# xingchensong/TouchNet

Hardware: AMD Instinct MI355X
Metric: audio+text tokens/sec/node (packed seq, full train step) + step MFU (higher is better)
Workload: dtype bf16

## Files before the change

### touchnet_amd/csrc/common.h

```cpp
#pragma once
#include <hip/hip_runtime.h>
#include <stdint.h>

#define TN_OK 0
#define TN_EINVAL (-22)

#define TN_LAUNCH_CHECK()                                   \
  do {                                                      \
    hipError_t e__ = hipGetLastError();                     \
    if (e__ != hipSuccess) return (int)e__;                 \
  } while (0)

namespace tn {

typedef uint16_t bf16_t;

typedef __attribute__((ext_vector_type(8))) __bf16 bf16x8_t;
typedef __attribute__((ext_vector_type(16))) float f32x16_t;
typedef __attribute__((ext_vector_type(4))) float f32x4_t;

__device__ __forceinline__ float bf2f(bf16_t v) { return __uint_as_float(((uint32_t)v) << 16); }

typedef __attribute__((ext_vector_type(2))) __bf16 bf16x2_t;

// ... 69 lines not shown
      f[2 * i + 1] = __uint_as_float(w[i] & 0xffff0000u);
    }
  }
  __device__ __forceinline__ void pack(const float (&f)[8]) {
    raw.x = pack2bf(f[0], f[1]);
    raw.y = pack2bf(f[2], f[3]);
    raw.z = pack2bf(f[4], f[5]);
    raw.w = pack2bf(f[6], f[7]);
  }
};
template <> struct Vec16<float> {
  static constexpr int N = 4;
  float4 raw;
  __device__ __forceinline__ void load(const float* p) { raw = *reinterpret_cast<const float4*>(p); }
  __device__ __forceinline__ void store(float* p) const { *reinterpret_cast<float4*>(p) = raw; }
  __device__ __forceinline__ void unpack(float (&f)[4]) const {
    f[0] = raw.x; f[1] = raw.y; f[2] = raw.z; f[3] = raw.w;
  }
  __device__ __forceinline__ void pack(const float (&f)[4]) { raw = make_float4(f[0], f[1], f[2], f[3]); }
};

__device__ __forceinline__ float wave_sum(float v) {
#pragma unroll
  for (int o = 32; o > 0; o >>= 1) v += __shfl_xor(v, o, 64);
  return v;
}
__device__ __forceinline__ float wave_max(float v) {
#pragma unroll
  for (int o = 32; o > 0; o >>= 1) v = fmaxf(v, __shfl_xor(v, o, 64));
  return v;
}

__device__ __forceinline__ float block_sum(float v, float* sm) {
  v = wave_sum(v);
  const int lane = threadIdx.x & 63, w = threadIdx.x >> 6, nw = (blockDim.x + 63) >> 6;
  __syncthreads();
  if (lane == 0) sm[w] = v;
  __syncthreads();
  float r = 0.f;
  for (int i = 0; i < nw; ++i) r += sm[i];
  return r;
}
__device__ __forceinline__ float block_max(float v, float* sm) {
  v = wave_max(v);
  const int lane = threadIdx.x & 63, w = threadIdx.x >> 6, nw = (blockDim.x + 63) >> 6;
  __syncthreads();
  if (lane == 0) sm[w] = v;
  __syncthreads();
  float r = sm[0];
  for (int i = 1; i < nw; ++i) r = fmaxf(r, sm[i]);
  return r;
}

}
```

### touchnet_amd/csrc/gemm.hip

```cpp
#include <stdlib.h>

#include <type_traits>
#include <utility>

#include "common.h"

namespace tn {
namespace gemm {

constexpr int BM = 256, BN = 256;
constexpr int SLOT = 32768;
constexpr int LDS_BYTES = 5 * SLOT;
constexpr int NT = 512;
constexpr int MAXSEG = 3;

typedef __attribute__((address_space(3))) void* lds_ptr_t;
typedef __attribute__((ext_vector_type(2))) uint32_t u32x2_t;
typedef __attribute__((ext_vector_type(4))) uint32_t u32x4_t;

struct Seg {
  const bf16_t* A;
  const bf16_t* B;
  long long lda, ldb;
  int K;
  int pad_;
};

struct Grp {
  bf16_t* C;
  long long ldc;
  int M, N, nbm, nbn;
  int start;
  int stages;
};

constexpr int EPI_PLAIN = 0, EPI_GROUPED = 1, EPI_SWIGLU_FWD = 2, EPI_SWIGLU_BWD = 3, EPI_BIASG = 4, EPI_ROPE = 5;
constexpr int EPI_GELU_FWD = 6, EPI_GELU_BWD = 7;

struct Params {
  Seg seg[MAXSEG];
  int nseg;
  int M, N;
  bf16_t* C;
  bf16_t* Ct;
  const bf16_t* bias;
  long long ldc, ldct;
  int accumulate;
  const bf16_t* addend;
  long long ldadd;
  int nbm, nbn;
  int stages;
  int splitk, kchunk;
  float* ws;
  int tile0, ntiles;
  int c_f32;
  Grp grp[MAXSEG];
  int ngrp;
  bf16_t* C2;
  bf16_t* C3;
  const bf16_t* E1;
  const bf16_t* E2;
  long long lde;
  bf16_t* bias_out;
  float* bias_ws;
  const bf16_t* rope_cos;
  const bf16_t* rope_sin;
  int rope_d;
};

__device__ __forceinline__ void tile_of_block(int bid, int nbm, int nbn, int& tm, int& tn) {
  const int total = nbm * nbn;
  const int xcd = bid & 7, local = bid >> 3;
  const int q = total >> 3, r = total & 7;
  const int vid = (xcd < r ? xcd * (q + 1) : r * (q + 1) + (xcd - r) * q) + local;
  constexpr int GM = 8;
  const int per_group = GM * nbn;
  const int g = vid / per_group, w = vid - g * per_group;
  const int gm = min(GM, nbm - g * GM);
  tm = g * GM + w % gm;
  tn = w / gm;
}

typedef f32x16_t Acc[4][2];

constexpr int kPieceB[4] = {0, 2, 4, 6}, kPieceA[4] = {14, 18, 22, 26};
static_assert(kPieceB[3] < kPieceA[0], "every B piece is issued before the first A piece");

template <bool IS_A> constexpr int piece_at(int pos) {
  for (int i = 0; i < 4; ++i)
    if ((IS_A ? kPieceA[i] : kPieceB[i]) == pos) return i;
  return -1;
}
constexpr int early_piece_count() {
  int n = 0;
  for (int i = 0; i < 4; ++i) n += (kPieceB[i] < 8) + (kPieceA[i] < 8);
  return n;
}

template <bool KMAJ, bool M16 = false>
struct Stream {
  __amdgpu_buffer_rsrc_t rs;
  int soff;
  int step;
  int left;
  int seg;
  int ld2;
  int voff[4];

  __device__ __forceinline__ void set_voff(int wave, int lane) {
    if constexpr (!KMAJ) {
#pragma unroll
      for (int q = 0; q < 4; ++q) {
        const int row = wave * 32 + q * 8 + (lane >> 3);
        voff[q] = row * ld2 + (((lane & 7) ^ ((row >> 1) & 7)) << 4);
      }
    } else {
#pragma unroll
      for (int q = 0; q < 4; ++q) {
        const int k = wave * 8 + q * 2 + (lane >> 5);
        const int u = lane & 31;
// ... 192 lines not shown
        if (sB.seg + 1 < p.nseg) open_b(sB.seg + 1);
        else if (++kb < mine) open_b(0);
        else sB.kill(p.C);
      }
    };
    auto piece_a = [&](int slot, int q) {
      __builtin_amdgcn_raw_ptr_buffer_load_lds(sA.rs, (lds_ptr_t)(smem + slot * SLOT + wave * 4096 + q * 1024), 16,
                                               sA.voff[q], sA.soff, 0, 0);
    };
    auto piece_b = [&](int slot, int q) {
      __builtin_amdgcn_raw_ptr_buffer_load_lds(sB.rs, (lds_ptr_t)(smem + slot * SLOT + wave * 4096 + q * 1024), 16,
                                               sB.voff[q], sB.soff, 0, 0);
    };
    open_a(0);
    open_b(0);

    Reader<AK, 4> ra(lane, wr * 128);
    Reader<BK, 2> rb(lane, wc * 64);

    Acc acc;
    auto zero_acc = [&]() {
#pragma unroll
      for (int i = 0; i < 4; ++i)
#pragma unroll
        for (int j = 0; j < 2; ++j)
#pragma unroll
          for (int r = 0; r < 16; ++r) acc[i][j][r] = 0.f;
    };
    zero_acc();

    Frags<AK, 4> ae, ao;
    Frags<BK, 2> be, bo;

#define TN_PIN() __builtin_amdgcn_sched_barrier(0)
    auto read_frag = [&](auto QC, auto FC, int sa, int sb, Frags<AK, 4>& a, Frags<BK, 2>& b) {
      constexpr int Q = decltype(QC)::value, F = decltype(FC)::value;
      if constexpr (F < 2) rb.template read<Q, F>(smem, sb * SLOT, b);
      else ra.template read<Q, F - 2>(smem, sa * SLOT, a);
    };
    auto read_all = [&](auto QC, int sa, int sb, Frags<AK, 4>& a, Frags<BK, 2>& b) {
      read_frag(QC, std::integral_constant<int, 0>{}, sa, sb, a, b);
      read_frag(QC, std::integral_constant<int, 1>{}, sa, sb, a, b);
      read_frag(QC, std::integral_constant<int, 2>{}, sa, sb, a, b);
      read_frag(QC, std::integral_constant<int, 3>{}, sa, sb, a, b);
      read_frag(QC, std::integral_constant<int, 4>{}, sa, sb, a, b);
      read_frag(QC, std::integral_constant<int, 5>{}, sa, sb, a, b);
    };
    auto mma = [&](const Frags<AK, 4>& a, const Frags<BK, 2>& b, int i, int j) {
      acc[i][j] = __builtin_amdgcn_mfma_f32_32x32x16_bf16(b.v[j], a.v[i], acc[i][j], 0, 0, 0);
    };

    float bsum = 0.f;
    bool bias_on = false;
    auto bias_accum = [&](const Frags<AK, 4>& a) {
      auto add = [&](const bf16x8_t& v) {
        const u32x4_t w = __builtin_bit_cast(u32x4_t, v);
        bsum += ((__uint_as_float(w.x << 16) + __uint_as_float(w.x & 0xffff0000u)) +
                 (__uint_as_float(w.y << 16) + __uint_as_float(w.y & 0xffff0000u))) +
                ((__uint_as_float(w.z << 16) + __uint_as_float(w.z & 0xffff0000u)) +
                 (__uint_as_float(w.w << 16) + __uint_as_float(w.w & 0xffff0000u)));
      };
      if (wc == 0) add(a.v[0]);
      else if (wc == 1) add(a.v[1]);
      else if (wc == 2) add(a.v[2]);
      else add(a.v[3]);
    };

    auto quarter = [&](auto NQC, auto P0C, const Frags<AK, 4>& ca, const Frags<BK, 2>& cb, Frags<AK, 4>& na,
                       Frags<BK, 2>& nb, int nsa, int nsb, int dst_b, int dst_a) {
      constexpr int P0 = decltype(P0C)::value;
      if constexpr (EPI == EPI_BIASG) {
        if (bias_on) bias_accum(ca);
        TN_PIN();
      }
      auto step = [&](auto MC) {
        constexpr int m = decltype(MC)::value;
        mma(ca, cb, m >> 1, m & 1);
        TN_PIN();
        if constexpr (m < 6) {
          read_frag(NQC, std::integral_constant<int, m>{}, nsa, nsb, na, nb);
          TN_PIN();
        }
        constexpr int pb = P0 < 0 ? -1 : piece_at<false>(P0 + m);
        constexpr int pa = P0 < 0 ? -1 : piece_at<true>(P0 + m);
        if constexpr (pb >= 0) {
          piece_b(dst_b, pb);
          if constexpr (pb == 3) adv_b();
          TN_PIN();
        }
        if constexpr (pa >= 0) {
          piece_a(dst_a, pa);
          if constexpr (pa == 3) adv_a();
          TN_PIN();
        }
      };
      step(std::integral_constant<int, 0>{});
      step(std::integral_constant<int, 1>{});
      step(std::integral_constant<int, 2>{});
      step(std::integral_constant<int, 3>{});
      step(std::integral_constant<int, 4>{});
      step(std::integral_constant<int, 5>{});
      step(std::integral_constant<int, 6>{});
      step(std::integral_constant<int, 7>{});
    };
    auto early_pieces = [&](int dst_b, int dst_a) {
      auto one = [&](auto MC) {
        constexpr int m = decltype(MC)::value;
        constexpr int pb = piece_at<false>(m), pa = piece_at<true>(m);
        if constexpr (pb >= 0) {
          piece_b(dst_b, pb);
          if constexpr (pb == 3) adv_b();
        }
        if constexpr (pa >= 0) {
          piece_a(dst_a, pa);
          if constexpr (pa == 3) adv_a();
        }
      };
      one(std::integral_constant<int, 0>{});
      one(std::integral_constant<int, 1>{});
      one(std::integral_constant<int, 2>{});
      one(std::integral_constant<int, 3>{});
      one(std::integral_constant<int, 4>{});
      one(std::integral_constant<int, 5>{});
      one(std::integral_constant<int, 6>{});
      one(std::integral_constant<int, 7>{});
    };
    auto next = [](int s, int d) { s += d; return s >= 5 ? s - 5 : s; };
    using I0 = std::integral_constant<int, 0>;
    using I1 = std::integral_constant<int, 1>;
    using I2 = std::integral_constant<int, 2>;
    using I3 = std::integral_constant<int, 3>;
    using NONE = std::integral_constant<int, -1>;

#pragma unroll
    for (int q = 0; q < 4; ++q) piece_a(0, q);
    adv_a();
#pragma unroll
    for (int q = 0; q < 4; ++q) piece_b(1, q);
    adv_b();
#pragma unroll
    for (int q = 0; q < 4; ++q) piece_a(2, q);
    adv_a();
    early_pieces(3, 4);
    asm volatile("s_waitcnt vmcnt(%0)" ::"n"(4 + early_piece_count()) : "memory");
    __builtin_amdgcn_s_barrier();
    int sa = 0, sb = 1;
    int pa = 4, pb = 3;

    auto trip = [&](auto LASTC) {
      constexpr bool LAST = decltype(LASTC)::value;
      const int sa1 = next(sa, 2), sb1 = next(sb, 2);
      __builtin_amdgcn_s_setprio(1);
      quarter(I1{}, std::integral_constant<int, 8>{}, ae, be, ao, bo, sa, sb, pb, pa);
      wait_frags(ao, bo);
      TN_PIN();
      quarter(I2{}, std::integral_constant<int, 16>{}, ao, bo, ae, be, sa, sb, pb, pa);
      wait_frags(ae, be);
      TN_PIN();
      quarter(I3{}, std::integral_constant<int, 24>{}, ae, be, ao, bo, sa, sb, pb, pa);
      __builtin_amdgcn_s_setprio(0);
      wait_frags(ao, bo);
      __builtin_amdgcn_s_waitcnt(0xc07f);
      asm volatile("s_waitcnt vmcnt(4)" ::: "memory");
      __builtin_amdgcn_s_barrier();
      __builtin_amdgcn_s_setprio(1);
      if constexpr (!LAST) {
        quarter(I0{}, I0{}, ao, bo, ae, be, sa1, sb1, sa, sb);
        __builtin_amdgcn_s_setprio(0);
        wait_frags(ae, be);
        TN_PIN();
      } else {
        if constexpr (EPI == EPI_BIASG) {
          if (bias_on) bias_accum(ao);
        }
#pragma unroll
        for (int m = 0; m < 8; ++m) mma(ao, bo, m >> 1, m & 1);
        __builtin_amdgcn_s_setprio(0);
      }
      pb = sa;
      pa = sb;
      sa = sa1;
      sb = sb1;
    };

    const int np_all = SPLITK ? p.kchunk : p.stages;
    for (int kc = 0; kc < mine; ++kc) {
      int np = np_all;
      if constexpr (EPI == EPI_BIASG) {
        int m0_, n0_, g_;
        origin_g(kc, m0_, n0_, g_);
        bias_on = n0_ == 0;
        bsum = 0.f;
      }
      if constexpr (EPI == EPI_GROUPED) {
        int m0_, n0_, g_;
        origin_g(kc, m0_, n0_, g_);
        np = p.grp[g_].stages;
      }
      read_all(I0{}, sa, sb, ae, be);
      wait_frags(ae, be);
      TN_PIN();
      for (int t = 1; t < np; ++t) trip(std::false_type{});
      trip(std::true_type{});
      int m0, n0, grp;
      origin_g(kc, m0, n0, grp);
      if constexpr (EPI == EPI_BIASG) {
        if (bias_on) {
          const float tot = bsum + __shfl_xor(bsum, 32, 64);
          const int m = m0 + wr * 128 + wc * 32 + (lane & 31);
          if (lane < 32) {
            if constexpr (SPLITK) {
              p.bias_ws[(long long)split_of(kc) * (p.nbm * BM) + m] = tot;
            } else if (m < p.M) {
              p.bias_out[m] = f2bf(tot);
            }
          }
        }
      }
      if constexpr (SPLITK) {
        const int u = bid + kc * G, sp = u / tiles;
        epilogue_ws(p, acc, sp * tiles + (u - sp * tiles), wr * 128, wc * 64, lane);
      } else if constexpr (OUT_F32) {
        if constexpr (EPI == EPI_GROUPED) {
          const Out o = {p.grp[grp].C, p.grp[grp].ldc, p.grp[grp].M, p.grp[grp].N};
          epilogue_f32(p, o, acc, m0 + wr * 128, n0 + wc * 64, lane);
        } else {
          const Out o = {p.C, p.ldc, p.M, p.N};
          epilogue_f32(p, o, acc, m0 + wr * 128, n0 + wc * 64, lane);
        }
      } else if constexpr (EPI == EPI_GROUPED) {
        const Out o = {p.grp[grp].C, p.grp[grp].ldc, p.grp[grp].M, p.grp[grp].N};
        epilogue(p, o, acc, smem + (wave < 4 ? pb : pa) * SLOT + (wave & 3) * 8192, m0 + wr * 128, n0 + wc * 64, lane);
      } else {
        const Out o = {p.C, p.ldc, p.M, p.N};
        epilogue(p, o, acc, smem + (wave < 4 ? pb : pa) * SLOT + (wave & 3) * 8192, m0 + wr * 128, n0 + wc * 64, lane);
      }
      zero_acc();
      __builtin_amdgcn_s_waitcnt(0xc07f);
      __builtin_amdgcn_s_barrier();
      asm volatile("" : "+v"(lane));
      ra = Reader<AK, 4>(lane, wr * 128);
      rb = Reader<BK, 2>(lane, wc * 64);
      sA.set_voff(wave, lane);
      sB.set_voff(wave, lane);
      early_pieces(pb, pa);
    }
  }

  static __device__ __forceinline__ void epilogue_f32(const Params& p, const Out& o, Acc& acc, int wm0, int wn0, int lane) {
    const int l31 = lane & 31, hi = lane >> 5;
    float* C = reinterpret_cast<float*>(o.C);
    const bool add = p.accumulate != 0;
#pragma unroll
    for (int i = 0; i < 4; ++i) {
      const int m = wm0 + i * 32 + l31;
#pragma unroll
      for (int j = 0; j < 2; ++j)
#pragma unroll
        for (int g = 0; g < 4; ++g) {
          const int n = wn0 + j * 32 + 8 * g + 4 * hi;
          if (m < o.M && n < o.N) {
            f32x4_t* dst = reinterpret_cast<f32x4_t*>(C + (long long)m * o.ldc + n);
            f32x4_t v = {acc[i][j][4 * g], acc[i][j][4 * g + 1], acc[i][j][4 * g + 2], acc[i][j][4 * g + 3]};
            if (add) v += *dst;
            *dst = v;
          }
        }
    }
  }

// ... 674 lines not shown
            float f[8], df[8];
            x.unpack(f);
            d.unpack(df);
#pragma unroll
            for (int e = 0; e < 8; e += 2) {
              const gelu_f32x2 r = gelu_grad_f2(gelu_f32x2{f[e], f[e + 1]}, gelu_f32x2{df[e], df[e + 1]});
              df[e] = r.x;
              df[e + 1] = r.y;
            }
            d.pack(df);
            *reinterpret_cast<uint4*>(dst) = d.raw;
            continue;
          }
          if (acc_c) {
            Vec16<bf16_t> o, nw;
            o.load(p.addend != nullptr ? p.addend + (long long)m * p.ldadd + n : dst);
            nw.raw = v;
            float fo[8], fn[8];
            o.unpack(fo);
            nw.unpack(fn);
#pragma unroll
            for (int e = 0; e < 8; ++e) fn[e] += fo[e];
            nw.pack(fn);
            v = nw.raw;
          }
          *reinterpret_cast<uint4*>(dst) = v;
        }
      }
    }
  }
};

template <bool AK, bool BK, int EPI = EPI_PLAIN>
__global__ __launch_bounds__(NT, 2) void gemm16_kernel(const Params p) {
  __shared__ __attribute__((aligned(1024))) char smem[LDS_BYTES];
  Kernel16<AK, BK, EPI>::run(p, smem);
}

__global__ __launch_bounds__(256) void splitk_reduce_kernel(const float* __restrict__ ws, int S, int M, int N, int nbm,
                                                            int nbn, int tile0, int ntiles, bf16_t* __restrict__ C,
                                                            long long ldc, const bf16_t* __restrict__ bias,
                                                            int accumulate, int out_f32,
                                                            const float* __restrict__ bias_ws,
                                                            bf16_t* __restrict__ bias_out) {
  const int t = blockIdx.x >> 5, part = blockIdx.x & 31;
  int tm, tn;
  tile_of_block(tile0 + t, nbm, nbn, tm, tn);
  const int idx = part * 256 + threadIdx.x;
  const int lm = idx >> 5, ln = (idx & 31) * 8;
  const int m = tm * BM + lm, n = tn * BN + ln;
  if (m >= M || n >= N) return;
  if (bias_out != nullptr && tn == 0 && ln == 0) {
    float b = 0.f;
    for (int sp = 0; sp < S; ++sp) b += bias_ws[(long long)sp * (nbm * BM) + m];
    bias_out[m] = f2bf(b);
  }
  float a[8] = {0.f, 0.f, 0.f, 0.f, 0.f, 0.f, 0.f, 0.f};
  const float* src = ws + (long long)t * (BM * BN) + lm * BN + ln;
  const long long slab = (long long)ntiles * (BM * BN);
  for (int sp = 0; sp < S; ++sp) {
    const float4 x = *reinterpret_cast<const float4*>(src + sp * slab);
    const float4 y = *reinterpret_cast<const float4*>(src + sp * slab + 4);
    a[0] += x.x; a[1] += x.y; a[2] += x.z; a[3] += x.w;
    a[4] += y.x; a[5] += y.y; a[6] += y.z; a[7] += y.w;
  }
  if (out_f32) {
    float* d = reinterpret_cast<float*>(C) + (long long)m * ldc + n;
    float4 x = make_float4(a[0], a[1], a[2], a[3]), y = make_float4(a[4], a[5], a[6], a[7]);
    if (accumulate) {
      const float4 ox = *reinterpret_cast<const float4*>(d), oy = *reinterpret_cast<const float4*>(d + 4);
      x.x += ox.x; x.y += ox.y; x.z += ox.z; x.w += ox.w;
      y.x += oy.x; y.y += oy.y; y.z += oy.z; y.w += oy.w;
    }
    *reinterpret_cast<float4*>(d) = x;
    *reinterpret_cast<float4*>(d + 4) = y;
    return;
  }
  bf16_t* dst = C + (long long)m * ldc + n;
  if (bias != nullptr) {
    Vec16<bf16_t> b;
    float fb[8];
    b.load(bias + n);
    b.unpack(fb);
#pragma unroll
    for (int e = 0; e < 8; ++e) a[e] += fb[e];
  }
  if (accumulate) {
    Vec16<bf16_t> o;
    float fo[8];
    o.load(dst);
    o.unpack(fo);
#pragma unroll
    for (int e = 0; e < 8; ++e) a[e] += fo[e];
  }
  Vec16<bf16_t> out;
  out.pack(a);
  out.store(dst);
}

template <bool AK, bool BK, bool HAS_CT>
static int launch(dim3 grid, hipStream_t st, const Params& p) {
  constexpr bool WGRAD = AK && BK && !HAS_CT;
  auto reduce = [&](const float* bias_ws, bf16_t* bias_out) {
    hipLaunchKernelGGL(splitk_reduce_kernel, dim3((unsigned)p.ntiles * 32u), dim3(256), 0, st, p.ws, p.splitk, p.M, p.N,
                       p.nbm, p.nbn, p.tile0, p.ntiles, p.C, p.ldc, p.bias, p.accumulate, p.c_f32, bias_ws, bias_out);
  };
  if (p.bias_out != nullptr) {
    if constexpr (WGRAD) {
      if (p.splitk > 1) {
        hipLaunchKernelGGL((gemm_kernel<true, true, false, true, false, EPI_BIASG>), grid, dim3(NT), 0, st, p);
        reduce(p.bias_ws, p.bias_out);
      } else if (p.c_f32) {
        hipLaunchKernelGGL((gemm_kernel<true, true, false, false, true, EPI_BIASG>), grid, dim3(NT), 0, st, p);
      } else {
        hipLaunchKernelGGL((gemm_kernel<true, true, false, false, false, EPI_BIASG>), grid, dim3(NT), 0, st, p);
      }
    } else {
      return -1;
    }
  } else if (p.splitk > 1) {
    if constexpr (!HAS_CT) {
      hipLaunchKernelGGL((gemm_kernel<AK, BK, false, true>), grid, dim3(NT), 0, st, p);
      reduce(nullptr, nullptr);
    } else {
      return -1;
    }
  } else if (p.c_f32) {
    if constexpr (WGRAD) {
      hipLaunchKernelGGL((gemm_kernel<true, true, false, false, true>), grid, dim3(NT), 0, st, p);
    } else {
      return -1;
    }
  } else if constexpr (!AK && !HAS_CT) {
    hipLaunchKernelGGL((gemm16_kernel<AK, BK>), grid, dim3(NT), 0, st, p);
  } else {
    hipLaunchKernelGGL((gemm_kernel<AK, BK, HAS_CT>), grid, dim3(NT), 0, st, p);
  }
  return 0;
}

}
}

extern "C" {

static int g_persistent = 1;
void tn_gemm_set_persistent(int on) { g_persistent = on ? 1 : 0; }
int tn_gemm_get_persistent(void) { return g_persistent; }

namespace {

int num_cus() {
  static const int ncu = [] {
    int dev = 0, n = 256;
    if (hipGetDevice(&dev) == hipSuccess) (void)hipDeviceGetAttribute(&n, hipDeviceAttributeMultiprocessorCount, dev);
    return n >= 8 ? n / 8 * 8 : 8;
  }();
  return ncu;
}

bool persistent_now() {
  const char* pe = getenv("TN_GEMM_PERSIST");
  return pe ? atoi(pe) != 0 : g_persistent != 0;
}

void clear_params(tn::gemm::Params& p) {
  p = tn::gemm::Params{};
  p.splitk = 1;
// ... 26 lines not shown
    if (k <= 0 || ((k % 64) != 0 && !(a_kmaj && b_kmaj)) || (lda[s] % 8) || (ldb[s] % 8)) return TN_EINVAL;
    if (((uintptr_t)A[s] | (uintptr_t)B[s]) & 15) return TN_EINVAL;
    if (a_kmaj) {
      if (lda[s] < M || ((long long)(k - 1) * lda[s] + M) * 2 >= 0x7fffffffLL) return TN_EINVAL;
    } else {
      if (lda[s] <= 0 || (long long)288 * lda[s] * 2 >= 0x7fffffffLL) return TN_EINVAL;
    }
    if (b_kmaj) {
      if (ldb[s] <= 0 || ((long long)(k - 1) * ldb[s] + N) * 2 >= 0x7fffffffLL) return TN_EINVAL;
    } else {
      if (ldb[s] <= 0 || (long long)288 * ldb[s] * 2 >= 0x7fffffffLL) return TN_EINVAL;
    }
    p.seg[s].A = (const tn::bf16_t*)A[s];
    p.seg[s].B = (const tn::bf16_t*)B[s];
    p.seg[s].lda = lda[s];
    p.seg[s].ldb = ldb[s];
    p.seg[s].K = k;
    p.seg[s].pad_ = 0;
    p.stages += (k + 63) / 64;
  }
  for (int s = nseg; s < MAXSEG; ++s) p.seg[s] = p.seg[0];
  if (Ct != nullptr && ((M % 8) || (ldct % 8) || ldct < M || ((uintptr_t)Ct & 15))) return TN_EINVAL;
  if (Ct != nullptr && accumulate) return TN_EINVAL;
  p.nseg = nseg;
  p.M = M;
  p.N = N;
  p.C = (tn::bf16_t*)C;
  p.Ct = (tn::bf16_t*)Ct;
  p.bias = (const tn::bf16_t*)bias;
  p.ldc = ldc;
  p.ldct = ldct;
  p.accumulate = accumulate;
  p.addend = (const tn::bf16_t*)addend;
  p.ldadd = ldadd;
  p.nbm = (M + BM - 1) / BM;
  p.nbn = (N + BN - 1) / BN;
  p.splitk = 1;
  p.kchunk = 0;
  p.ws = nullptr;
  p.tile0 = 0;
  p.ntiles = p.nbm * p.nbn;
  p.c_f32 = c_f32;
  const int ncu = num_cus();
  int main_tiles = 0;
  if (splitk > 1) {
    if (nseg != 1 || Ct != nullptr) return TN_EINVAL;
    if (!(a_kmaj && b_kmaj) && (p.stages % splitk) != 0) return TN_EINVAL;
    if (tail_only) {
      main_tiles = p.ntiles / ncu * ncu;
      if (main_tiles <= 0 || main_tiles >= p.ntiles) return TN_EINVAL;
    }
    const long long slabs = (long long)splitk * (p.ntiles - main_tiles) * BM * BN;
    if (workspace == nullptr || ((uintptr_t)workspace & 15) ||
        workspace_bytes < (slabs + (bias_grad ? (long long)splitk * p.nbm * BM : 0)) * (long long)sizeof(float))
      return TN_EINVAL;
    p.splitk = splitk;
    p.kchunk = (p.stages + splitk - 1) / splitk;
    p.ws = (float*)workspace;
    p.bias_ws = bias_grad ? (float*)workspace + slabs : nullptr;
  }
  p.bias_out = (tn::bf16_t*)bias_grad;
  const bool persist = persistent_now();
  hipStream_t st = (hipStream_t)stream;
  int rc = 0;
#define TN_MODE(AKM, BKM, GRID, PRM) \
  rc |= (Ct != nullptr) ? launch<AKM, BKM, true>(GRID, st, PRM) : launch<AKM, BKM, false>(GRID, st, PRM)
#define TN_LAUNCH(GRID, PRM)                                                               \
  if (!a_kmaj && !b_kmaj) TN_MODE(false, false, GRID, PRM);                                \
  else if (!a_kmaj && b_kmaj) TN_MODE(false, true, GRID, PRM);                             \
  else if (a_kmaj && b_kmaj) TN_MODE(true, true, GRID, PRM);                               \
  else return TN_EINVAL
  if (main_tiles > 0) {
    Params pm = p;
    pm.splitk = 1;
    pm.ntiles = main_tiles;
    const dim3 gm(ncu);
    TN_LAUNCH(gm, pm);
    p.tile0 = main_tiles;
    p.ntiles -= main_tiles;
  }
  {
    const int units = p.ntiles * p.splitk;
    const dim3 grid(persist && units > ncu ? ncu : units);
    TN_LAUNCH(grid, p);
  }
#undef TN_LAUNCH
#undef TN_MODE
  if (rc != 0) return TN_EINVAL;
  TN_LAUNCH_CHECK();
  return TN_OK;
}

int tn_gemm_bf16(const void* const* A, const void* const* B, const long long* lda, const long long* ldb, const int* K,
                 int nseg, int a_kmaj, int b_kmaj, void* C, void* Ct, const void* bias, int M, int N, long long ldc,
                 long long ldct, int accumulate, void* stream) {
  return gemm_launch(A, B, lda, ldb, K, nseg, a_kmaj, b_kmaj, C, Ct, bias, M, N, ldc, ldct, accumulate, 1, 0, nullptr, 0,
                     stream);
}

int tn_gemm_bf16_addend(const void* A, const void* B, long long lda, long long ldb, int K, int a_kmaj, int b_kmaj, void* C,
                        const void* bias, const void* addend, long long ldadd, int M, int N, long long ldc, void* stream) {
  if (addend == nullptr || addend == C) return TN_EINVAL;
  return gemm_launch(&A, &B, &lda, &ldb, &K, 1, a_kmaj, b_kmaj, C, nullptr, bias, M, N, ldc, 0, 0, 1, 0, nullptr, 0, stream,
                     0, nullptr, addend, ldadd);
}

int tn_gemm_bf16_splitk(const void* A, const void* B, long long lda, long long ldb, int K, int a_kmaj, int b_kmaj,
                        void* C, const void* bias, int M, int N, long long ldc, int accumulate, int splitk, int tail_only,
                        void* workspace, long long workspace_bytes, void* stream) {
  if (splitk < 2) return TN_EINVAL;
  return gemm_launch(&A, &B, &lda, &ldb, &K, 1, a_kmaj, b_kmaj, C, nullptr, bias, M, N, ldc, 0, accumulate, splitk,
                     tail_only, workspace, workspace_bytes, stream);
// ... 307 lines not shown
```

### touchnet_amd/csrc/norm_act.hip

```cpp
#include "common.h"

namespace tn {

constexpr int kRowWaves = 4;

template <typename T, int MAXV>
__global__ __launch_bounds__(256) void rmsnorm_fwd_kernel(const T* __restrict__ x, const T* __restrict__ res_in,
                                                          const T* __restrict__ w, T* __restrict__ y,
                                                          T* __restrict__ res_out, float* __restrict__ rstd_out,
                                                          int rows, int H, float eps) {
  constexpr int N = Vec16<T>::N;
  const int lane = threadIdx.x & 63;
  const int row = blockIdx.x * kRowWaves + (threadIdx.x >> 6);
  if (row >= rows) return;
  const int nvec = H / N;
  const size_t base = (size_t)row * H;
  float hv[MAXV][N];
  float ss = 0.f;
#pragma unroll
  for (int i = 0; i < MAXV; ++i) {
    const int v = i * 64 + lane;
    if (v < nvec) {
      Vec16<T> a;
      a.load(x + base + (size_t)v * N);
// ... 109 lines not shown
      if (v < nvec) {
        float o[N];
#pragma unroll
        for (int j = 0; j < N; ++j) o[j] = rstd * (g[i][j] - xh[i][j] * dot);
        if (dres) {
          Vec16<T> r;
          float rf[N];
          r.load(dres + base + (size_t)v * N);
          r.unpack(rf);
#pragma unroll
          for (int j = 0; j < N; ++j) o[j] += rf[j];
        }
        Vec16<T> ov;
        ov.pack(o);
        ov.store(dh + base + (size_t)v * N);
      }
    }
  }
#pragma unroll
  for (int i = 0; i < MAXV; ++i) {
    const int v = i * 256 + tid;
    if (v < nvec) {
#pragma unroll
      for (int j = 0; j < N; ++j) dw_partial[(size_t)blockIdx.x * H + v * N + j] = dwacc[i][j];
    }
  }
}

template <typename T>
__global__ __launch_bounds__(256) void colsum_partials_kernel(const float* __restrict__ partial, T* __restrict__ out,
                                                              int P, int H) {
  __shared__ float sm[16][16 + 1];
  const int cx = threadIdx.x & 15, ry = threadIdx.x >> 4;
  const int c = blockIdx.x * 16 + cx;
  float s0 = 0.f, s1 = 0.f, s2 = 0.f, s3 = 0.f;
  if (c < H) {
    int p = ry;
    for (; p + 48 < P; p += 64) {
      s0 += partial[(size_t)p * H + c];
      s1 += partial[(size_t)(p + 16) * H + c];
      s2 += partial[(size_t)(p + 32) * H + c];
      s3 += partial[(size_t)(p + 48) * H + c];
    }
    for (; p < P; p += 16) s0 += partial[(size_t)p * H + c];
  }
  sm[ry][cx] = (s0 + s1) + (s2 + s3);
  __syncthreads();
  if (ry == 0 && c < H) {
    float t = 0.f;
#pragma unroll
    for (int k = 0; k < 16; ++k) t += sm[k][cx];
    Elem<T>::st(out + c, t);
  }
}

__global__ __launch_bounds__(256) void colsum_rows_kernel(const bf16_t* __restrict__ x, float* __restrict__ partial,
                                                          int rows, int cols, long long ld, int rps) {
  __shared__ float sm[8][256 + 8];
  const int cx = threadIdx.x & 31, ry = threadIdx.x >> 5;
  const int c0 = blockIdx.x * 256 + cx * 8;
  const int r_beg = blockIdx.y * rps, r_end = min(r_beg + rps, rows);
  float acc[8] = {0.f, 0.f, 0.f, 0.f, 0.f, 0.f, 0.f, 0.f};
  if (c0 < cols) {
    for (int r = r_beg + ry; r < r_end; r += 8) {
      Vec16<bf16_t> v;
      float f[8];
      v.load(x + (size_t)r * ld + c0);
      v.unpack(f);
#pragma unroll
      for (int j = 0; j < 8; ++j) acc[j] += f[j];
    }
  }
#pragma unroll
  for (int j = 0; j < 8; ++j) sm[ry][cx * 8 + j] = acc[j];
  __syncthreads();
  const int c = blockIdx.x * 256 + threadIdx.x;
  if (c < cols) {
    float t = 0.f;
#pragma unroll
    for (int k = 0; k < 8; ++k) t += sm[k][threadIdx.x];
    partial[(size_t)blockIdx.y * cols + c] = t;
  }
}

template <typename T, int MAXV>
__global__ __launch_bounds__(256) void layernorm_fwd_kernel(const T* __restrict__ x, const T* __restrict__ res_in,
                                                            const T* __restrict__ w, const T* __restrict__ b,
                                                            T* __restrict__ y, T* __restrict__ res_out,
                                                            float* __restrict__ mean_out, float* __restrict__ rstd_out,
                                                            int rows, int H, float eps) {
  constexpr int N = Vec16<T>::N;
  const int lane = threadIdx.x & 63;
  const int row = blockIdx.x * kRowWaves + (threadIdx.x >> 6);
  if (row >= rows) return;
  const int nvec = H / N;
  const size_t base = (size_t)row * H;
  float hv[MAXV][N];
  float s = 0.f;
#pragma unroll
  for (int i = 0; i < MAXV; ++i) {
    const int v = i * 64 + lane;
    if (v < nvec) {
      Vec16<T> a;
      a.load(x + base + (size_t)v * N);
      a.unpack(hv[i]);
      if (res_in) {
// ... 643 lines not shown
```

### touchnet_amd/functional.py

```python
from __future__ import annotations

import math
import os
from dataclasses import dataclass
from typing import Optional

import torch

from . import _C
from . import library as L

_cur = _C.stream
_p = _C.ptr


def _c(t: torch.Tensor) -> torch.Tensor:
    return t if t.is_contiguous() else t.contiguous()


def rms_norm(x, weight, eps, residual=None):
    y, h, _ = L.rmsnorm_fwd(x, residual, weight, float(eps))
    return (y, h) if residual is not None else y


# ... 335 lines not shown
    if a.dim() != 2 or b.dim() != 2 or a.dtype != torch.bfloat16 or b.dtype != torch.bfloat16:
        raise _C.KernelError("gemm_tn: 2-D bf16 operands only")
    if a.stride(1) != 1 or b.stride(1) != 1 or a.shape[1] != b.shape[1]:
        raise _C.KernelError("gemm_tn: operands must be contraction-contiguous [M, K] / [N, K]")
    M, K = a.shape
    N = b.shape[0]
    if out is None:
        if accumulate:
            raise _C.KernelError("gemm_tn: accumulate needs `out`")
        out = torch.empty(M, N, dtype=a.dtype, device=a.device)
    if out.stride(1) != 1 or tuple(out.shape) != (M, N):
        raise _C.KernelError("gemm_tn: bad `out`")
    if bias is not None:
        bias = _c(bias).to(a.dtype)
    _C.check(_C.lib().tn_gemm_bf16_tn(_p(a), _p(b), _p(out), _p(out_t), _p(bias), M, N, K, a.stride(0), b.stride(0),
                                      out.stride(0), out_t.stride(0) if out_t is not None else 0, int(accumulate),
                                      _cur()), "tn_gemm_bf16_tn")
    return out


def gemm(segs, a_kmaj: bool = False, b_kmaj: bool = False, bias: Optional[torch.Tensor] = None,
         out: Optional[torch.Tensor] = None, accumulate: bool = False,
         out_t: Optional[torch.Tensor] = None, bias_grad: Optional[torch.Tensor] = None,
         addend: Optional[torch.Tensor] = None) -> torch.Tensor:
    if not 1 <= len(segs) <= 3:
        raise _C.KernelError("gemm: 1..3 segments")
    for a, b in segs:
        if a.dim() != 2 or b.dim() != 2 or a.dtype != torch.bfloat16 or b.dtype != torch.bfloat16:
            raise _C.KernelError("gemm: 2-D bf16 operands only")
        if a.stride(1) != 1 or b.stride(1) != 1:
            raise _C.KernelError("gemm: operands need contiguous rows")
    a0, b0 = segs[0]
    M = a0.shape[1] if a_kmaj else a0.shape[0]
    N = b0.shape[1] if b_kmaj else b0.shape[0]
    Ks = []
    for a, b in segs:
        Ka, Ma = (a.shape[0], a.shape[1]) if a_kmaj else (a.shape[1], a.shape[0])
        Kb, Nb = (b.shape[0], b.shape[1]) if b_kmaj else (b.shape[1], b.shape[0])
        if Ka != Kb or Ma != M or Nb != N:
            raise _C.KernelError(f"gemm: segment shapes disagree: a {tuple(a.shape)} b {tuple(b.shape)}")
        Ks.append(Ka)
    if out is None:
        if accumulate:
            raise _C.KernelError("gemm: accumulate needs `out`")
        out = torch.empty(M, N, dtype=torch.bfloat16, device=a0.device)
    if out.dtype == torch.float32:
        if not (a_kmaj and b_kmaj and len(segs) == 1 and bias is None and out_t is None):
            raise _C.KernelError("gemm: fp32 output exists for the single-segment weight-gradient mode only")
        if out.stride(1) != 1 or tuple(out.shape) != (M, N) or not a0.is_cuda:
            raise _C.KernelError("gemm: bad fp32 `out`")
        split = split_k(M, N, Ks[0], True, True) if SPLIT_K else 1
        ws = None
        if split > 1:
            ws = torch.empty(split * (((M + 255) // 256) * ((N + 255) // 256) * 65536 + (M + 255) // 256 * 256),
                             dtype=torch.float32, device=a0.device)
        if bias_grad is not None:
            _check_bias_grad(bias_grad, M, a0)
            _C.check(_C.lib().tn_gemm_bf16_wgrad_bias(_p(a0), _p(b0), a0.stride(0), b0.stride(0), Ks[0], _p(out), _p(bias_grad),
                                                      M, N, out.stride(0), int(accumulate), 1, split, _p(ws),
                                                      ws.numel() * 4 if ws is not None else 0, _cur()),
                     "tn_gemm_bf16_wgrad_bias")
            return out
        _C.check(_C.lib().tn_gemm_bf16_wgrad_f32(_p(a0), _p(b0), a0.stride(0), b0.stride(0), Ks[0], _p(out), M, N,
                                                 out.stride(0), int(accumulate), split, _p(ws),
                                                 ws.numel() * 4 if ws is not None else 0, _cur()), "tn_gemm_bf16_wgrad_f32")
        return out
    if out.stride(1) != 1 or tuple(out.shape) != (M, N) or out.dtype != torch.bfloat16:
        raise _C.KernelError("gemm: bad `out`")
    if bias is not None:
        bias = _c(bias).to(torch.bfloat16)
    n = len(segs)
    if not a0.is_cuda:
        raise _C.KernelError("touchnet_amd kernels need device (HIP) tensors; got a CPU tensor")
    if addend is not None:
        if (n != 1 or accumulate or out_t is not None or bias_grad is not None or addend.dtype != torch.bfloat16
                or tuple(addend.shape) != (M, N) or addend.stride(1) != 1 or addend.data_ptr() == out.data_ptr()):
            raise _C.KernelError("gemm: addend needs one segment, a bf16 [M, N] matrix with contiguous rows that is not `out`")
        _C.check(_C.lib().tn_gemm_bf16_addend(_p(a0), _p(b0), a0.stride(0), b0.stride(0), Ks[0], int(a_kmaj), int(b_kmaj),
                                              _p(out), _p(bias), _p(addend), addend.stride(0), M, N, out.stride(0), _cur()),
                 "tn_gemm_bf16_addend")
        return out
    split = 1
    if bias_grad is not None:
        if not (a_kmaj and b_kmaj and n == 1 and bias is None and out_t is None):
            raise _C.KernelError("gemm: bias_grad exists for the single-segment weight-gradient mode only")
        _check_bias_grad(bias_grad, M, a0)
        split = split_k(M, N, Ks[0], True, True) if SPLIT_K else 1
        ws = None
        if split > 1:
            ws = torch.empty(split * (((M + 255) // 256) * ((N + 255) // 256) * 65536 + (M + 255) // 256 * 256),
                             dtype=torch.float32, device=a0.device)
        _C.check(_C.lib().tn_gemm_bf16_wgrad_bias(_p(a0), _p(b0), a0.stride(0), b0.stride(0), Ks[0], _p(out), _p(bias_grad), M,
                                                  N, out.stride(0), int(accumulate), 0, split, _p(ws),
                                                  ws.numel() * 4 if ws is not None else 0, _cur()), "tn_gemm_bf16_wgrad_bias")
        return out
    if n == 1 and out_t is None and SPLIT_K:
        split = split_k(M, N, Ks[0], a_kmaj, b_kmaj)
    if split > 1:
        tiles = ((M + 255) // 256) * ((N + 255) // 256)
        ws = torch.empty(split * tiles * 65536, dtype=torch.float32, device=a0.device)
        _C.check(_C.lib().tn_gemm_bf16_splitk(_p(a0), _p(b0), a0.stride(0), b0.stride(0), Ks[0], int(a_kmaj), int(b_kmaj),
                                              _p(out), _p(bias), M, N, out.stride(0), int(accumulate), split, 0,
                                              _p(ws), ws.numel() * 4, _cur()), "tn_gemm_bf16_splitk")
        return out
    import ctypes as C
    Ap = (C.c_void_p * n)(*[a.data_ptr() for a, _ in segs])
    Bp = (C.c_void_p * n)(*[b.data_ptr() for _, b in segs])
    la = (C.c_longlong * n)(*[a.stride(0) for a, _ in segs])
    lb = (C.c_longlong * n)(*[b.stride(0) for _, b in segs])
    Kc = (C.c_int * n)(*Ks)
    _C.check(_C.lib().tn_gemm_bf16(Ap, Bp, la, lb, Kc, n, int(a_kmaj), int(b_kmaj), _p(out), _p(out_t), _p(bias), M, N,
                                   out.stride(0), out_t.stride(0) if out_t is not None else 0, int(accumulate),
                                   _cur()), "tn_gemm_bf16")
    return out


def _check_bias_grad(bias_grad, M, like):
    if (bias_grad.dtype != torch.bfloat16 or bias_grad.dim() != 1 or bias_grad.numel() != M or not bias_grad.is_contiguous()
            or bias_grad.device != like.device):
        raise _C.KernelError("gemm: bias_grad must be a contiguous bf16 [M] device vector")


def gemm_grouped_wgrad(pairs, outs=None, accumulate: bool = False):
    import ctypes as C
    n = len(pairs)
    if not 1 <= n <= 3:
        raise _C.KernelError("gemm_grouped_wgrad: 1..3 products")
    for a, b in pairs:
        if (a.dim() != 2 or b.dim() != 2 or a.dtype != torch.bfloat16 or b.dtype != torch.bfloat16 or a.stride(1) != 1
                or b.stride(1) != 1 or a.shape[0] != b.shape[0] or not a.is_cuda):
            raise _C.KernelError("gemm_grouped_wgrad: pairs of 2-D bf16 device matrices [K, M] / [K, N] with contiguous rows")
    if outs is None:
        if accumulate:
            raise _C.KernelError("gemm_grouped_wgrad: accumulate needs `outs`")
        outs = [torch.empty(a.shape[1], b.shape[1], dtype=torch.bfloat16, device=a.device) for a, b in pairs]
    f32 = outs[0].dtype == torch.float32
    for o, (a, b) in zip(outs, pairs):
        if (o.dtype != outs[0].dtype or o.dtype not in (torch.float32, torch.bfloat16) or o.stride(1) != 1
                or tuple(o.shape) != (a.shape[1], b.shape[1])):
            raise _C.KernelError("gemm_grouped_wgrad: bad `outs`")
    Ms = (C.c_int * n)(*[a.shape[1] for a, _ in pairs])
    Ns = (C.c_int * n)(*[b.shape[1] for _, b in pairs])
    Ks = (C.c_int * n)(*[a.shape[0] for a, _ in pairs])
    need = int(_C.lib().tn_gemm_grouped_workspace_bytes(Ms, Ns, Ks, n))
    ws = torch.empty(need // 4, dtype=torch.float32, device=outs[0].device) if need > 0 else None
    Ap = (C.c_void_p * n)(*[a.data_ptr() for a, _ in pairs])
    Bp = (C.c_void_p * n)(*[b.data_ptr() for _, b in pairs])
    Cp = (C.c_void_p * n)(*[o.data_ptr() for o in outs])
    la = (C.c_longlong * n)(*[a.stride(0) for a, _ in pairs])
    lb = (C.c_longlong * n)(*[b.stride(0) for _, b in pairs])
    lc = (C.c_longlong * n)(*[o.stride(0) for o in outs])
    _C.check(_C.lib().tn_gemm_bf16_grouped(Ap, Bp, la, lb, Ks, Cp, lc, Ms, Ns, n, 1, 1, int(accumulate), int(f32), _p(ws),
                                           need, _cur()), "tn_gemm_bf16_grouped")
    return list(outs)


def gemm_swiglu_fwd(x2: torch.Tensor, w_gate: torch.Tensor, w_up: torch.Tensor):
    M, K = x2.shape
    I = w_gate.shape[0]
    if not _bf16_rows(x2, w_gate, w_up) or w_up.shape != w_gate.shape or w_gate.shape[1] != K or w_gate.stride(0) != w_up.stride(0):
        raise _C.KernelError("gemm_swiglu_fwd: bf16 device matrices x [M, K], w_gate / w_up [I, K] of one row pitch")
    gate, up, act = (torch.empty(M, I, dtype=torch.bfloat16, device=x2.device) for _ in range(3))
    _C.check(_C.lib().tn_gemm_bf16_swiglu_fwd(_p(x2), _p(w_gate), _p(w_up), _p(gate), _p(up), _p(act), M, I, K, x2.stride(0),
                                              w_gate.stride(0), I, _cur()), "tn_gemm_bf16_swiglu_fwd")
    return gate, up, act


# ... 799 lines not shown
```

Baseline: 22640.

## Spread wgrad bias-gradient row sums across all N tiles with partial reduction

Before, the fused bias-gradient in the weight-gradient GEMM was accumulated only by the tiles at n0 == 0, which put the whole row-sum work on one column of tiles. Now each tile sums a rotating share of the K stages, chosen by its column index, and writes a float partial per N tile into a workspace. A separate column-sum kernel, or the split-K reduce, then adds the partials. This evens out the per-tile epilogue load at the cost of a larger workspace, an extra kernel launch and an extra allocation on the non-split path.

```diff
diff --git a/touchnet_amd/csrc/common.h b/touchnet_amd/csrc/common.h
--- a/touchnet_amd/csrc/common.h
+++ b/touchnet_amd/csrc/common.h
@@ -145,4 +145,6 @@
   return r;
 }
 
+void colsum_partials_bf16(const float* partial, bf16_t* out, int P, int H, hipStream_t st);
+
 }
diff --git a/touchnet_amd/csrc/gemm.hip b/touchnet_amd/csrc/gemm.hip
--- a/touchnet_amd/csrc/gemm.hip
+++ b/touchnet_amd/csrc/gemm.hip
@@ -66,6 +66,7 @@
   const bf16_t* rope_cos;
   const bf16_t* rope_sin;
   int rope_d;
+  int bias_ld;
 };
 
 __device__ __forceinline__ void tile_of_block(int bid, int nbm, int nbn, int& tm, int& tn) {
@@ -364,6 +365,7 @@
 
     float bsum = 0.f;
     bool bias_on = false;
+    int bias_turn = 0;
     auto bias_accum = [&](const Frags<AK, 4>& a) {
       auto add = [&](const bf16x8_t& v) {
         const u32x4_t w = __builtin_bit_cast(u32x4_t, v);
@@ -462,6 +464,10 @@
     auto trip = [&](auto LASTC) {
       constexpr bool LAST = decltype(LASTC)::value;
       const int sa1 = next(sa, 2), sb1 = next(sb, 2);
+      if constexpr (EPI == EPI_BIASG) {
+        bias_on = bias_turn == 0;
+        bias_turn = bias_on ? p.nbn - 1 : bias_turn - 1;
+      }
       __builtin_amdgcn_s_setprio(1);
       quarter(I1{}, std::integral_constant<int, 8>{}, ae, be, ao, bo, sa, sb, pb, pa);
       wait_frags(ao, bo);
@@ -501,7 +507,7 @@
       if constexpr (EPI == EPI_BIASG) {
         int m0_, n0_, g_;
         origin_g(kc, m0_, n0_, g_);
-        bias_on = n0_ == 0;
+        bias_turn = n0_ / BN;
         bsum = 0.f;
       }
       if constexpr (EPI == EPI_GROUPED) {
@@ -517,17 +523,10 @@
       int m0, n0, grp;
       origin_g(kc, m0, n0, grp);
       if constexpr (EPI == EPI_BIASG) {
-        if (bias_on) {
-          const float tot = bsum + __shfl_xor(bsum, 32, 64);
-          const int m = m0 + wr * 128 + wc * 32 + (lane & 31);
-          if (lane < 32) {
-            if constexpr (SPLITK) {
-              p.bias_ws[(long long)split_of(kc) * (p.nbm * BM) + m] = tot;
-            } else if (m < p.M) {
-              p.bias_out[m] = f2bf(tot);
-            }
-          }
-        }
+        const float tot = bsum + __shfl_xor(bsum, 32, 64);
+        const int m = m0 + wr * 128 + wc * 32 + (lane & 31);
+        const int slot = (SPLITK ? split_of(kc) * p.nbn : 0) + n0 / BN;
+        if (lane < 32 && m < p.bias_ld) p.bias_ws[(long long)slot * p.bias_ld + m] = tot;
       }
       if constexpr (SPLITK) {
         const int u = bid + kc * G, sp = u / tiles;
@@ -1308,7 +1307,7 @@
   if (m >= M || n >= N) return;
   if (bias_out != nullptr && tn == 0 && ln == 0) {
     float b = 0.f;
-    for (int sp = 0; sp < S; ++sp) b += bias_ws[(long long)sp * (nbm * BM) + m];
+    for (int sp = 0; sp < S * nbn; ++sp) b += bias_ws[(long long)sp * (nbm * BM) + m];
     bias_out[m] = f2bf(b);
   }
   float a[8] = {0.f, 0.f, 0.f, 0.f, 0.f, 0.f, 0.f, 0.f};
@@ -1366,10 +1365,12 @@
       if (p.splitk > 1) {
         hipLaunchKernelGGL((gemm_kernel<true, true, false, true, false, EPI_BIASG>), grid, dim3(NT), 0, st, p);
         reduce(p.bias_ws, p.bias_out);
-      } else if (p.c_f32) {
-        hipLaunchKernelGGL((gemm_kernel<true, true, false, false, true, EPI_BIASG>), grid, dim3(NT), 0, st, p);
       } else {
-        hipLaunchKernelGGL((gemm_kernel<true, true, false, false, false, EPI_BIASG>), grid, dim3(NT), 0, st, p);
+        if (p.c_f32)
+          hipLaunchKernelGGL((gemm_kernel<true, true, false, false, true, EPI_BIASG>), grid, dim3(NT), 0, st, p);
+        else
+          hipLaunchKernelGGL((gemm_kernel<true, true, false, false, false, EPI_BIASG>), grid, dim3(NT), 0, st, p);
+        colsum_partials_bf16(p.bias_ws, p.bias_out, p.nbn, p.M, st);
       }
     } else {
       return -1;
@@ -1502,12 +1503,19 @@
     }
     const long long slabs = (long long)splitk * (p.ntiles - main_tiles) * BM * BN;
     if (workspace == nullptr || ((uintptr_t)workspace & 15) ||
-        workspace_bytes < (slabs + (bias_grad ? (long long)splitk * p.nbm * BM : 0)) * (long long)sizeof(float))
+        workspace_bytes < (slabs + (bias_grad ? (long long)splitk * p.ntiles * BM : 0)) * (long long)sizeof(float))
       return TN_EINVAL;
     p.splitk = splitk;
     p.kchunk = (p.stages + splitk - 1) / splitk;
     p.ws = (float*)workspace;
     p.bias_ws = bias_grad ? (float*)workspace + slabs : nullptr;
+    p.bias_ld = p.nbm * BM;
+  } else if (bias_grad != nullptr) {
+    if (workspace == nullptr || ((uintptr_t)workspace & 3) ||
+        workspace_bytes < (long long)p.nbn * M * (long long)sizeof(float))
+      return TN_EINVAL;
+    p.bias_ws = (float*)workspace;
+    p.bias_ld = M;
   }
   p.bias_out = (tn::bf16_t*)bias_grad;
   const bool persist = persistent_now();
diff --git a/touchnet_amd/csrc/norm_act.hip b/touchnet_amd/csrc/norm_act.hip
--- a/touchnet_amd/csrc/norm_act.hip
+++ b/touchnet_amd/csrc/norm_act.hip
@@ -185,6 +185,10 @@
     for (int k = 0; k < 16; ++k) t += sm[k][cx];
     Elem<T>::st(out + c, t);
   }
+}
+
+void colsum_partials_bf16(const float* partial, bf16_t* out, int P, int H, hipStream_t st) {
+  hipLaunchKernelGGL((colsum_partials_kernel<bf16_t>), dim3((H + 15) / 16), dim3(256), 0, st, partial, out, P, H);
 }
 
 __global__ __launch_bounds__(256) void colsum_rows_kernel(const bf16_t* __restrict__ x, float* __restrict__ partial,
diff --git a/touchnet_amd/functional.py b/touchnet_amd/functional.py
--- a/touchnet_amd/functional.py
+++ b/touchnet_amd/functional.py
@@ -411,10 +411,11 @@
         split = split_k(M, N, Ks[0], True, True) if SPLIT_K else 1
         ws = None
         if split > 1:
-            ws = torch.empty(split * (((M + 255) // 256) * ((N + 255) // 256) * 65536 + (M + 255) // 256 * 256),
-                             dtype=torch.float32, device=a0.device)
+            ws = torch.empty(_wgrad_ws_floats(M, N, split, bias_grad is not None), dtype=torch.float32, device=a0.device)
         if bias_grad is not None:
             _check_bias_grad(bias_grad, M, a0)
+            if ws is None:
+                ws = torch.empty(_wgrad_ws_floats(M, N, 1, True), dtype=torch.float32, device=a0.device)
             _C.check(_C.lib().tn_gemm_bf16_wgrad_bias(_p(a0), _p(b0), a0.stride(0), b0.stride(0), Ks[0], _p(out), _p(bias_grad),
                                                       M, N, out.stride(0), int(accumulate), 1, split, _p(ws),
                                                       ws.numel() * 4 if ws is not None else 0, _cur()),
@@ -445,13 +446,10 @@
             raise _C.KernelError("gemm: bias_grad exists for the single-segment weight-gradient mode only")
         _check_bias_grad(bias_grad, M, a0)
         split = split_k(M, N, Ks[0], True, True) if SPLIT_K else 1
-        ws = None
-        if split > 1:
-            ws = torch.empty(split * (((M + 255) // 256) * ((N + 255) // 256) * 65536 + (M + 255) // 256 * 256),
-                             dtype=torch.float32, device=a0.device)
+        ws = torch.empty(_wgrad_ws_floats(M, N, split, True), dtype=torch.float32, device=a0.device)
         _C.check(_C.lib().tn_gemm_bf16_wgrad_bias(_p(a0), _p(b0), a0.stride(0), b0.stride(0), Ks[0], _p(out), _p(bias_grad), M,
-                                                  N, out.stride(0), int(accumulate), 0, split, _p(ws),
-                                                  ws.numel() * 4 if ws is not None else 0, _cur()), "tn_gemm_bf16_wgrad_bias")
+                                                  N, out.stride(0), int(accumulate), 0, split, _p(ws), ws.numel() * 4, _cur()),
+                 "tn_gemm_bf16_wgrad_bias")
         return out
     if n == 1 and out_t is None and SPLIT_K:
         split = split_k(M, N, Ks[0], a_kmaj, b_kmaj)
@@ -472,6 +470,13 @@
                                    out.stride(0), out_t.stride(0) if out_t is not None else 0, int(accumulate),
                                    _cur()), "tn_gemm_bf16")
     return out
+
+
+def _wgrad_ws_floats(M, N, split, bias_grad):
+    nbm, nbn = (M + 255) // 256, (N + 255) // 256
+    if split > 1:
+        return split * nbm * nbn * (65536 + (256 if bias_grad else 0))
+    return nbn * M if bias_grad else 0
 
 
 def _check_bias_grad(bias_grad, M, like):
```

After: 22240. 0.983x the previous value.
